# YzM1a0/MuDPT

Hardware: AMD Instinct MI355X
Metric: images/sec fwd+bwd ViT-B/16 MuDPT (higher is better)
Workload: dtype bf16; 1 GPU; MuDPT ViT-B/16 fwd+bwd+SGD, batch 256/GPU, 11 class prompts, n_ctx 4, depth 12, synthetic 224x224 N(0,1) images, random-init frozen CLIP (BASELINE configs[1]); global_batch=256, parallelism=dp1

## Files before the change

### include/mudpt.h

```cpp
#ifndef MUDPT_H
#define MUDPT_H

#include <stddef.h>
#include <stdint.h>

#ifdef __cplusplus
extern "C" {
#endif

#define MUDPT_ABI_VERSION 7

#define MUDPT_OK 0
#define MUDPT_ERR_ARG 1
#define MUDPT_ERR_HIP 2
#define MUDPT_ERR_STATE 3

#define MUDPT_BF16 0
#define MUDPT_F16 1
#define MUDPT_F32 2

#define MUDPT_VARIANT_MUDPT 0
#define MUDPT_VARIANT_COCOOP 1
#define MUDPT_VARIANT_COOP 2
#define MUDPT_VARIANT_COOP_CSC 3
// ... 141 lines not shown
int mudpt_cocoop_dbias(int32_t dtype, const float* dx_f32, const void* dx_lp, float* dbias, int32_t B, int32_t C, int32_t L, int32_t d,
                       int32_t n, float scale, void* stream);
int mudpt_coop_dctx(int32_t dtype, const float* dx_f32, const void* dx_lp, const int32_t* rows, float* dctx, int32_t C, int32_t n, int32_t d,
                    int32_t csc, float scale, void* stream);
int mudpt_sgemm(int32_t transA, int32_t transB, int32_t M, int32_t N, int32_t K, float alpha, const float* A, int32_t lda,
                const float* B, int32_t ldb, float beta, float* C, int32_t ldc, const float* bias, void* stream);

int mudpt_layernorm_bwd_ex(int32_t dtype, const void* dy, int32_t lddy, int32_t dy_f32, const float* x, int32_t ldx, const int32_t* row_index,
                           const float* mean, const float* rstd, const float* gamma, const float* dres, const void* dres_lp, int32_t lddres,
                           float* dx, int32_t lddx, void* dx_lp, int32_t lddx_lp, float* side, int32_t side_row0, int32_t side_n, int32_t side_L,
                           size_t side_ldb, int32_t index_mode, int32_t rows, int32_t d, void* stream);
int mudpt_layernorm_fwd_ex(int32_t dtype, const float* x, int32_t ldx, const int32_t* row_index, const float* add, const void* add_lp, int32_t ldadd,
                           const float* ov_rows, int32_t ov_row0, int32_t ov_n, int32_t ov_L, float* xout, int32_t ldxout, const float* gamma,
                           const float* beta, void* out, void* out_lo, int32_t lo_mode, int32_t ldo, int32_t out_f32, float* mean, float* rstd,
                           int32_t rows, int32_t d, void* stream);
int mudpt_attention_fwd_split(int32_t dtype, const void* qkv, void* out, void* out_lo, int32_t lo_mode, int32_t ld_out, float* lse, int32_t B, int32_t L,
                              int32_t H, int32_t causal, void* stream);
int mudpt_attention_fwd_single_split(int32_t dtype, const void* qkv, const void* q_sel, const int32_t* sel_rows, void* out_sel, void* out_lo,
                                     int32_t lo_mode, int32_t ld_out, float* lse_sel, int32_t B, int32_t L, int32_t H, int32_t causal, void* stream);
int mudpt_attention_bwd_sel(int32_t dtype, const void* qkv, const void* out, const void* dout, const float* lse, float* delta, void* dqkv,
                            const int32_t* sel_rows, int32_t B, int32_t L, int32_t H, int32_t causal, void* stream);
int mudpt_head_ex(const float* img, const float* txt, const int64_t* labels, float scale, float grad_scale, int32_t B, int32_t B_total, int32_t C,
                  int32_t e, float* txt_n, float* txt_inv, float* logits, float* loss, float* row_loss, float* dimg, float* dtxt, int32_t path,
                  int32_t* path_taken, void* stream);
int mudpt_pair_head(const float* img, const float* txt, const int64_t* labels, float scale, float grad_scale, int32_t B, int32_t B_total, int32_t C,
                    int32_t e, float* logits, float* loss, float* row_loss, float* dtxt, void* stream);
int mudpt_patchify(int32_t dtype, const float* images, void* patches, void* patches_lo, int32_t lo_mode, int32_t B, int32_t image_size, int32_t patch,
                   int32_t ldk, void* stream);
int mudpt_set_rows(float* x, int32_t B, int32_t L, int32_t d, int32_t row0, int32_t n, const float* rows, const float* add, void* stream);
int mudpt_gather_rows(const void* src, size_t src_stride, const int32_t* rows, void* dst, size_t dst_stride, int32_t nrows, int32_t row_bytes, void* stream);
// ... 31 lines not shown
```

### mudpt_amd/capi.py

```python
from __future__ import annotations

import ctypes as C
import os
import re

HERE = os.path.dirname(os.path.abspath(__file__))
LIB_PATH = os.environ.get("MUDPT_LIB") or os.path.join(HERE, "lib", "libmudpt_hip.so")
HEADER_PATH = os.path.join(os.path.dirname(HERE), "include", "mudpt.h")

BF16, F16, F32 = 0, 1, 2
VARIANT_MUDPT, VARIANT_COCOOP, VARIANT_COOP, VARIANT_COOP_CSC, VARIANT_VPT, VARIANT_MPT, VARIANT_UMUDPT, VARIANT_UUMUDPT = 0, 1, 2, 3, 4, 5, 6, 7
CLASS_TOKEN_END, CLASS_TOKEN_MIDDLE, CLASS_TOKEN_FRONT = 0, 1, 2
ABI_VERSION = 7
EPI_STORE, EPI_GELU, EPI_RESIDUAL, EPI_GELU_BWD, EPI_PATCH, EPI_STORE_F32 = range(6)
ATTN_FORMS = ("FWD_PAIR", "FWD_PERSISTENT", "FWD_RESIDENT", "FWD_STAGED", "BWD_TWO", "BWD_FUSED_W2", "BWD_FUSED_W1", "BWD_SWEEP", "BWD_RESIDENT",
              "BWD_STAGED")
GEMM_FORMS = ("PP", "T256x256", "T128x256", "T256x128", "T64x64_K128", "T64x64", "T128x64_RING4", "T128x128", "SPLITK_K128", "SPLITK_K64")


class MudptError(RuntimeError):
    pass


class Config(C.Structure):
# ... 55 lines not shown
    "mudpt_attention_fwd_exact": (_i32, [_vp, _vp, _vp, _vp, _i32, _i32, _vp, _i32, _i32, _i32, _i32, _vp]),
    "mudpt_attention_bwd": (_i32, [_i32, _vp, _vp, _vp, _vp, _vp, _vp, _i32, _i32, _i32, _i32, _vp]),
    "mudpt_attention_fwd_single": (_i32, [_i32, _vp, _vp, _vp, _vp, _vp, _i32, _i32, _i32, _i32, _vp]),
    "mudpt_attention_bwd_single": (_i32, [_i32, _vp, _vp, _vp, _vp, _vp, _vp, _vp, _vp, _i32, _i32, _i32, _i32, _vp]),
    "mudpt_layernorm_fwd_fused": (_i32, [_i32, _vp, _i32, _vp, _vp, _i32, _vp, _i32, _i32, _i32, _vp, _i32, _vp, _vp, _vp, _i32, _i32,
                                         _vp, _vp, _i32, _i32, _vp]),
    "mudpt_head": (_i32, [_vp, _vp, _vp, _f32, _f32, _i32, _i32, _i32, _vp, _vp, _vp, _vp, _vp]),
    "mudpt_reduce_rows": (_i32, [_i32, _vp, _vp, _i32, _i32, _i32, _i32, _i32, _vp, _i32, _i32, _f32, _vp]),
    "mudpt_cocoop_dbias": (_i32, [_i32, _vp, _vp, _vp, _i32, _i32, _i32, _i32, _i32, _f32, _vp]),
    "mudpt_coop_dctx": (_i32, [_i32, _vp, _vp, _vp, _vp, _i32, _i32, _i32, _i32, _f32, _vp]),
    "mudpt_sgemm": (_i32, [_i32, _i32, _i32, _i32, _i32, _f32, _vp, _i32, _vp, _i32, _f32, _vp, _i32, _vp, _vp]),
    "mudpt_layernorm_bwd_ex": (_i32, [_i32, _vp, _i32, _i32, _vp, _i32, _vp, _vp, _vp, _vp, _vp, _vp, _i32, _vp, _i32, _vp, _i32,
                                      _vp, _i32, _i32, _i32, _sz, _i32, _i32, _i32, _vp]),
    "mudpt_layernorm_fwd_ex": (_i32, [_i32, _vp, _i32, _vp, _vp, _vp, _i32, _vp, _i32, _i32, _i32, _vp, _i32, _vp, _vp, _vp, _vp, _i32, _i32, _i32,
                                      _vp, _vp, _i32, _i32, _vp]),
    "mudpt_attention_fwd_split": (_i32, [_i32, _vp, _vp, _vp, _i32, _i32, _vp, _i32, _i32, _i32, _i32, _vp]),
    "mudpt_attention_fwd_single_split": (_i32, [_i32, _vp, _vp, _vp, _vp, _vp, _i32, _i32, _vp, _i32, _i32, _i32, _i32, _vp]),
    "mudpt_attention_bwd_sel": (_i32, [_i32, _vp, _vp, _vp, _vp, _vp, _vp, _vp, _i32, _i32, _i32, _i32, _vp]),
    "mudpt_head_ex": (_i32, [_vp, _vp, _vp, _f32, _f32, _i32, _i32, _i32, _i32, _vp, _vp, _vp, _vp, _vp, _vp, _vp, _i32, C.POINTER(_i32), _vp]),
    "mudpt_pair_head": (_i32, [_vp, _vp, _vp, _f32, _f32, _i32, _i32, _i32, _i32, _vp, _vp, _vp, _vp, _vp]),
    "mudpt_patchify": (_i32, [_i32, _vp, _vp, _vp, _i32, _i32, _i32, _i32, _i32, _vp]),
    "mudpt_set_rows": (_i32, [_vp, _i32, _i32, _i32, _i32, _i32, _vp, _vp, _vp]),
    "mudpt_gather_rows": (_i32, [_vp, _sz, _vp, _vp, _sz, _i32, _i32, _vp]),
    "mudpt_scatter_rows": (_i32, [_vp, _sz, _vp, _vp, _sz, _i32, _i32, _vp]),
    "mudpt_add_rows": (_i32, [_i32, _vp, _vp, _vp, _i32, _i32, _vp]),
    "mudpt_linear_bwd": (_i32, [_i32, _i32, _i32, _vp, _vp, _vp, _vp, _vp, _vp, _vp]),
    "mudpt_colsum": (_i32, [_vp, _i32, _i32, _i32, _vp, _i32, _vp]),
    "mudpt_add": (_i32, [_vp, _vp, _vp, _sz, _vp]),
    "mudpt_cast": (_i32, [_i32, _vp, _vp, _sz, _vp]),
    "mudpt_relu": (_i32, [_vp, _sz, _vp]),
# ... 68 lines not shown
```

### mudpt_amd/csrc/common.h

```cpp
#pragma once
#include <hip/hip_runtime.h>
#include <hip/hip_ext.h>
#include <stdint.h>

#include "../../include/mudpt.h"

namespace mudpt {

typedef __attribute__((ext_vector_type(8))) __bf16 bf16x8;
typedef __attribute__((ext_vector_type(4))) __bf16 bf16x4;
typedef __attribute__((ext_vector_type(8))) _Float16 f16x8;
typedef __attribute__((ext_vector_type(4))) _Float16 f16x4;
typedef __attribute__((ext_vector_type(4))) float f32x4;
typedef __attribute__((ext_vector_type(16))) float f32x16;
typedef __attribute__((ext_vector_type(8))) int i32x8;

enum DType : int { DT_BF16 = 0, DT_F16 = 1 };

struct BF16 {
    using elem = __bf16;
    using vec8 = bf16x8;
    using vec4 = bf16x4;
    static constexpr int id = DT_BF16;
    __device__ static inline f32x4 mfma16(vec8 a, vec8 b, f32x4 c) {
// ... 71 lines not shown
}

template <int CTRL, int ROW_MASK = 0xf>
__device__ inline float dpp_mov(float v, float old) {
    return __builtin_bit_cast(float, __builtin_amdgcn_update_dpp(__builtin_bit_cast(int, old), __builtin_bit_cast(int, v), CTRL, ROW_MASK, 0xf, false));
}
__device__ inline float wave_sum(float v) {
    v += dpp_mov<0xb1>(v, 0.f);
    v += dpp_mov<0x4e>(v, 0.f);
    v += dpp_mov<0x141>(v, 0.f);
    v += dpp_mov<0x140>(v, 0.f);
    v += dpp_mov<0x142, 0xa>(v, 0.f);
    v += dpp_mov<0x143, 0xc>(v, 0.f);
    return __builtin_bit_cast(float, __builtin_amdgcn_readlane(__builtin_bit_cast(int, v), 63));
}
__device__ inline float wave_max(float v) {
    v = fmaxf(v, dpp_mov<0xb1>(v, v));
    v = fmaxf(v, dpp_mov<0x4e>(v, v));
    v = fmaxf(v, dpp_mov<0x141>(v, v));
    v = fmaxf(v, dpp_mov<0x140>(v, v));
    v = fmaxf(v, dpp_mov<0x142, 0xa>(v, v));
    v = fmaxf(v, dpp_mov<0x143, 0xc>(v, v));
    return __builtin_bit_cast(float, __builtin_amdgcn_readlane(__builtin_bit_cast(int, v), 63));
}

__device__ inline int xcd_remap(int bid, int nwg) {
    const int q = nwg >> 3, r = nwg & 7, x = bid & 7;
    return (x < r ? x * (q + 1) : r * (q + 1) + (x - r) * q) + (bid >> 3);
}

// ... 53 lines not shown
```

### mudpt_amd/csrc/kernels.h

```cpp
#pragma once
#include "common.h"

namespace mudpt {

enum Epilogue : int {
    EPI_STORE = 0,
    EPI_GELU = 1,
    EPI_RESIDUAL = 2,
    EPI_GELU_BWD = 3,
    EPI_PATCH = 4,
    EPI_STORE_F32 = 5
};

struct GemmArgs {
    const void* A = nullptr;
    const void* B = nullptr;
    int M = 0, N = 0, K = 0, lda = 0, ldb = 0;
    const float* bias = nullptr;
    void* out0 = nullptr; int ldo0 = 0;
    void* out1 = nullptr; int ldo1 = 0;
    void* out1_lo = nullptr;
    int out1_lo_mode = LO_F16;
    const void* A_lo = nullptr; int lo_mode = LO_NONE;
    const void* B8 = nullptr; int b8_scale = 127;
// ... 22 lines not shown
int launch_gemm_pp(int dtype, int epi, const GemmArgs& a, hipStream_t s, const GemmOpts& o);

struct LnFwdArgs {
    const float* x = nullptr; int ldx = 0;
    const int* row_index = nullptr;
    const float* gamma = nullptr; const float* beta = nullptr;
    void* out = nullptr; int ldo = 0;
    void* out_lo = nullptr;
    int lo_mode = LO_F16;
    float* mean = nullptr; float* rstd = nullptr;
    int rows = 0, d = 0; bool out_f32 = false;
    const float* add = nullptr; int ldadd = 0;
    const void* add_lp = nullptr;
    float* xout = nullptr; int ldxout = 0;
    const float* ov_rows = nullptr; int ov_row0 = 0, ov_n = 0, ov_L = 1;
};
int launch_ln_fwd(int dtype, const LnFwdArgs& a, hipStream_t s, const LaunchProf* prof = nullptr);

struct LnBwdArgs {
    const void* dy = nullptr; int lddy = 0; bool dy_f32 = false;
    const float* x = nullptr; int ldx = 0;
    const int* row_index = nullptr;
    const float* mean = nullptr; const float* rstd = nullptr; const float* gamma = nullptr;
    const float* dres = nullptr; int lddres = 0;
    const void* dres_lp = nullptr;
    float* dx = nullptr; int lddx = 0;
    void* dx_lp = nullptr; int lddx_lp = 0;
    int rows = 0, d = 0;
    bool by_token = false;
    bool stats_by_token = false;
// ... 130 lines not shown
```

### mudpt_amd/csrc/layernorm.hip

```cpp
#include "kernels.h"

namespace mudpt {

constexpr int LN_MAXV = 4;

template <typename T, bool OUT_F32>
__global__ __launch_bounds__(256) void ln_fwd_kernel(LnFwdArgs p) {
    using elem = typename T::elem;
    const int lane = threadIdx.x & 63;
    const int r = blockIdx.x * 4 + (threadIdx.x >> 6);
    if (r >= p.rows) return;
    const size_t xr = p.row_index ? (size_t)p.row_index[r] : (size_t)r;
    const f32x4* x = (const f32x4*)(p.x + xr * p.ldx);
    const int d4 = p.d >> 2;
    f32x4 v[LN_MAXV];
    float s = 0.f;
    const f32x4* ov = nullptr;
    if (p.ov_rows) {
        const int pos = r % p.ov_L - p.ov_row0;
        if (pos >= 0 && pos < p.ov_n) ov = (const f32x4*)(p.ov_rows + (size_t)pos * p.d);
    }
    const f32x4* add = (p.add && !ov) ? (const f32x4*)(p.add + xr * p.ldadd) : nullptr;
    const typename T::vec4* add_lp = (p.add_lp && !ov) ? (const typename T::vec4*)((const elem*)p.add_lp + xr * p.ldadd) : nullptr;
#pragma unroll
// ... 106 lines not shown
            for (int j = 0; j < 4; ++j) dx[j] = rstd * (g[k][j] - c1 - xh[k][j] * c2);
            if (p.dres) dx += ((const f32x4*)(p.dres + t * p.lddres))[i];
            if (p.dres_lp) {
                dx += f32x4{(float)rv[k][0], (float)rv[k][1], (float)rv[k][2], (float)rv[k][3]};
            }
            if (side_row) { side_row[i] = dx; dx = f32x4{0.f, 0.f, 0.f, 0.f}; }
            if (p.dx) ((f32x4*)(p.dx + t * p.lddx))[i] = dx;
            if (p.dx_lp) {
                typename T::vec4 o = {(elem)dx[0], (elem)dx[1], (elem)dx[2], (elem)dx[3]};
                ((typename T::vec4*)((elem*)p.dx_lp + t * p.lddx_lp))[i] = o;
            }
        }
    }
}

int launch_ln_fwd(int dtype, const LnFwdArgs& a, hipStream_t s, const LaunchProf* prof) {
    ARG_CHECK(a.x && a.gamma && a.beta && a.out, "ln_fwd: null operand");
    ARG_CHECK(a.rows > 0 && a.d > 0 && a.d % 4 == 0 && a.d <= 256 * LN_MAXV, "ln_fwd: bad shape rows=%d d=%d", a.rows, a.d);
    ARG_CHECK(a.ldx % 4 == 0 && a.ldo % 4 == 0 && a.ldx >= a.d && a.ldo >= a.d, "ln_fwd: bad strides %d/%d", a.ldx, a.ldo);
    ARG_CHECK(!(a.add || a.add_lp) || (a.ldadd % 4 == 0 && a.ldadd >= a.d), "ln_fwd: bad addend stride %d", a.ldadd);
    ARG_CHECK(!a.xout || (a.ldxout % 4 == 0 && a.ldxout >= a.d), "ln_fwd: bad xout stride %d", a.ldxout);
    ARG_CHECK(!a.ov_rows || (a.ov_L > 0 && a.ov_row0 >= 0 && a.ov_n >= 0 && a.ov_row0 + a.ov_n <= a.ov_L),
              "ln_fwd: bad splice rows %d..+%d of %d", a.ov_row0, a.ov_n, a.ov_L);
    ARG_CHECK(!a.row_index || !(a.add || a.add_lp || a.xout || a.ov_rows), "ln_fwd: the fused add / splice / xout need the identity row map");
    ARG_CHECK(!a.out_lo || (!a.out_f32 && (a.lo_mode == LO_F16 || a.lo_mode == LO_F8)), "ln_fwd: out_lo needs a T output and lo_mode 1 / 2");
    const dim3 grid((a.rows + 3) / 4), block(256);
    if (dtype == DT_BF16) {
        if (a.out_f32) MUDPT_LAUNCH((ln_fwd_kernel<BF16, true>), grid, block, 0, s, prof, a);
        else MUDPT_LAUNCH((ln_fwd_kernel<BF16, false>), grid, block, 0, s, prof, a);
    } else if (dtype == DT_F16) {
        if (a.out_f32) MUDPT_LAUNCH((ln_fwd_kernel<F16, true>), grid, block, 0, s, prof, a);
        else MUDPT_LAUNCH((ln_fwd_kernel<F16, false>), grid, block, 0, s, prof, a);
    } else {
        set_error("ln_fwd: unknown dtype %d", dtype);
        return MUDPT_ERR_ARG;
    }
    HIP_TRY(hipGetLastError());
    return MUDPT_OK;
}

int launch_ln_bwd(int dtype, const LnBwdArgs& a, hipStream_t s, const LaunchProf* prof) {
    ARG_CHECK(a.dy && a.x && a.mean && a.rstd && a.gamma && (a.dx || a.dx_lp), "ln_bwd: null operand");
    ARG_CHECK(!(a.dres && a.dres_lp), "ln_bwd: dres and dres_lp are exclusive");
    ARG_CHECK(!a.side || (!a.row_index && a.side_L > 0 && a.side_n > 0), "ln_bwd: the fused splice backward needs the identity row map");
    ARG_CHECK(a.rows > 0 && a.d > 0 && a.d % 4 == 0 && a.d <= 256 * LN_MAXV, "ln_bwd: bad shape rows=%d d=%d", a.rows, a.d);
    ARG_CHECK(a.ldx % 4 == 0 && a.lddy % 4 == 0 && a.lddx % 4 == 0, "ln_bwd: strides must be multiples of 4");
    ARG_CHECK(a.ldx >= a.d && a.lddy >= a.d && (!a.dx || a.lddx >= a.d), "ln_bwd: a row stride is shorter than d=%d (%d/%d/%d)", a.d, a.ldx, a.lddy, a.lddx);
    ARG_CHECK(!(a.dres || a.dres_lp) || (a.lddres % 4 == 0 && a.lddres >= a.d), "ln_bwd: bad dres stride %d", a.lddres);
    ARG_CHECK(!a.dx_lp || (a.lddx_lp % 4 == 0 && a.lddx_lp >= a.d), "ln_bwd: bad dx_lp stride %d", a.lddx_lp);
    ARG_CHECK(!a.side || (a.side_row0 >= 0 && a.side_row0 + a.side_n <= a.side_L && a.side_ldb % 4 == 0 && a.side_ldb >= (size_t)a.side_n * a.d),
              "ln_bwd: bad splice rows %d..+%d of %d / side stride %zu", a.side_row0, a.side_n, a.side_L, a.side_ldb);
    const dim3 grid((a.rows + 3) / 4), block(256);
    if (dtype == DT_BF16) {
        if (a.dy_f32) MUDPT_LAUNCH((ln_bwd_kernel<BF16, true>), grid, block, 0, s, prof, a);
        else MUDPT_LAUNCH((ln_bwd_kernel<BF16, false>), grid, block, 0, s, prof, a);
    } else if (dtype == DT_F16) {
        if (a.dy_f32) MUDPT_LAUNCH((ln_bwd_kernel<F16, true>), grid, block, 0, s, prof, a);
        else MUDPT_LAUNCH((ln_bwd_kernel<F16, false>), grid, block, 0, s, prof, a);
    } else {
        set_error("ln_bwd: unknown dtype %d", dtype);
        return MUDPT_ERR_ARG;
    }
    HIP_TRY(hipGetLastError());
    return MUDPT_OK;
}

}
```

### mudpt_amd/csrc/model.cpp

```cpp
#include <dlfcn.h>
#include <stdarg.h>
#include <stdio.h>
#include <string.h>

#include <algorithm>
#include <cmath>
#include <string>
#include <vector>

#include "../../include/mudpt.h"
#include "kernels.h"

namespace mudpt {

static thread_local char g_err[1024] = "";
void set_error(const char* fmt, ...) {
    va_list ap;
    va_start(ap, fmt);
    vsnprintf(g_err, sizeof(g_err), fmt, ap);
    va_end(ap);
}
const char* get_error() { return g_err; }

static inline uint16_t f32_to_bf16(float f) {
// ... 946 lines not shown
    if (m_fc != LO_NONE) { l2.out_lo = t.h_sel_lo; l2.lo_mode = m_fc; }
    TRY(launch_ln_fwd(dt, l2, s));
    GemmArgs f; f.A = t.h_sel; f.lda = d; f.B = w.w_fc; f.ldb = d; f.M = S; f.N = 4 * d; f.K = d; f.bias = w.b_fc;
    split_operand(f, m_fc, t.h_sel_lo, w.w_fc8, w.s_fc8);
    f.out0 = t.u_sel; f.ldo0 = 4 * d; f.out1 = t.g_sel; f.ldo1 = 4 * d;
    f.gelu_q8 = m->gelu_q8 && t.split == LO_NONE;
    if (m_proj != LO_NONE) { f.out1_lo = t.g_sel_lo; f.out1_lo_mode = m_proj; }
    TRY(gemm_call(m, EPI_GELU, f, s));
    GemmArgs p; p.A = t.g_sel; p.lda = 4 * d; p.B = w.w_proj; p.ldb = 4 * d; p.M = S; p.N = d; p.K = 4 * d; p.bias = w.b_proj;
    split_operand(p, m_proj, t.g_sel_lo, w.w_proj8, w.s_proj8);
    p.out0 = t.xout_sel; p.ldo0 = d; p.aux = t.xmid_sel; p.ldaux = d;
    TRY(gemm_call(m, EPI_RESIDUAL, p, s));
    return MUDPT_OK;
}

static int block_fwd(mudpt_model* m, Tower& t, int i, int nseq, const float* splice, hipStream_t s) {
    const int M = tower_rows(t, nseq), d = t.d, dt = m->dtype, n = t.n;
    const std::vector<Tower::Seg> segs = tower_segs(t, nseq);
    const bool lp = m->lp_upd;
    BlockW& w = t.w[i];
    BlockAct& a = t.a[i];
    const size_t esz = 2;
    const int m_qkv = site_mode(t, SITE_QKV, d), m_out = site_mode(t, SITE_OUT, d), m_fc = site_mode(t, SITE_FC, d), m_proj = site_mode(t, SITE_PROJ, 4 * d);
    LnFwdArgs l1; l1.x = a.x_in; l1.ldx = d; l1.gamma = w.ln1_g; l1.beta = w.ln1_b; l1.out = t.h; l1.ldo = d; l1.mean = a.mean1; l1.rstd = a.rstd1; l1.rows = M; l1.d = d;
    if (m_qkv != LO_NONE) { l1.out_lo = t.h_lo; l1.lo_mode = m_qkv; }
    if (i > 0) {
        l1.x = t.a[i - 1].x_mid; l1.ldadd = d; l1.xout = a.x_in; l1.ldxout = d;
        if (lp) l1.add_lp = t.upd; else l1.add = t.upd;
        if (splice) { l1.ov_rows = splice; l1.ov_row0 = t.prompt_row0; l1.ov_n = n; l1.ov_L = t.L; }
    }
    if (splice && i > 0 && segs.size() > 1) {
        for (const Tower::Seg& g : segs) {
            LnFwdArgs b = l1;
            const size_t r0 = (size_t)g.row0;
            b.x = l1.x + r0 * l1.ldx; b.xout = l1.xout + r0 * l1.ldxout;
            if (l1.add) b.add = l1.add + r0 * l1.ldadd;
            if (l1.add_lp) b.add_lp = (const char*)l1.add_lp + r0 * l1.ldadd * esz;
            b.out = (char*)l1.out + r0 * l1.ldo * esz;
            if (l1.out_lo) b.out_lo = (char*)l1.out_lo + r0 * l1.ldo * esz;
            b.mean = l1.mean + r0; b.rstd = l1.rstd + r0; b.rows = g.nseq * g.L; b.ov_L = g.L;
            TRY(ln_fwd_call(m, t, b, s));
        }
    } else {
        TRY(ln_fwd_call(m, t, l1, s));
    }
    if (i + 1 == t.layers && m->last_single && !t.exact_attn && t.tail_rows) {
// ... 190 lines not shown
    const mudpt_config& c = m->cfg;
    const int dv = c.v_width, e = c.embed_dim, n = m->vis.n, D1 = m->vis.D1;
    const int P = (c.image_size / c.patch) * (c.image_size / c.patch), Lv = m->vis.L, K0 = (3 * c.patch * c.patch + 63) / 64 * 64;
    const PromptRoute pr = prompt_route(m, m->vis);
    const int m_patch = site_mode(m->vis, SITE_PATCH, K0);
    if (m_patch != LO_NONE) TRY(launch_patchify_split(m->dtype, images, m->patches, m->patches_lo, m_patch, B, c.image_size, c.patch, K0, s));
    else TRY(launch_patchify(m->dtype, images, m->patches, B, c.image_size, c.patch, K0, s));
    GemmArgs pe; pe.A = m->patches; pe.lda = K0; pe.B = m->conv_w; pe.ldb = K0; pe.M = B * P; pe.N = dv; pe.K = K0; pe.out0 = m->xpre; pe.ldo0 = dv;
    split_operand(pe, m_patch, m->patches_lo, m->conv_w8, m->conv_s8);
    pe.patches = P; pe.seq_len = Lv; pe.pos = m->vpos;
    TRY(gemm_call(m, EPI_PATCH, pe, s));
    TRY(launch_set_rows(m->xpre, B, Lv, dv, 0, 1, m->cls, m->vpos, s));
    if (n > 0) TRY(launch_set_rows(m->xpre, B, Lv, dv, Lv - n, n, pr.in0, pr.in0_add, s));
    LnFwdArgs lp; lp.x = m->xpre; lp.ldx = dv; lp.gamma = m->ln_pre_g; lp.beta = m->ln_pre_b; lp.out = m->vis.a[0].x_in; lp.ldo = dv; lp.out_f32 = true;
    lp.mean = m->pre_mean; lp.rstd = m->pre_rstd; lp.rows = B * Lv; lp.d = dv;
    TRY(launch_ln_fwd(m->dtype, lp, s));
    for (int i = 0; i < m->vis.layers; ++i) {
        TRY(block_fwd(m, m->vis, i, B, (i >= 1 && i - 1 < D1) ? pr.deep + (size_t)(i - 1) * n * dv : nullptr, s));
    }
    LnFwdArgs lq; lq.x = m->vis.xout_sel; lq.ldx = dv; lq.gamma = m->ln_post_g; lq.beta = m->ln_post_b; lq.out = m->f_ln; lq.ldo = dv;
    lq.out_f32 = true; lq.mean = m->post_mean; lq.rstd = m->post_rstd; lq.rows = B; lq.d = dv;
    TRY(launch_ln_fwd(m->dtype, lq, s));
    TRY(launch_sgemm(false, false, B, e, dv, 1.f, m->f_ln, dv, m->vproj, e, 0.f, m->img_f, e, nullptr, s));
    return MUDPT_OK;
}

static int cocoop_text_chunk(mudpt_model* m, int i0, int nb, hipStream_t s) {
    const mudpt_config& c = m->cfg;
    const int dt = c.t_width, e = c.embed_dim, n = c.n_ctx, C = c.n_cls, Lt = m->txt.L, TS = nb * C;
    const size_t r0 = (size_t)i0 * C;
    TRY(launch_cocoop_prompts(m->txt.a[0].x_in, m->emb_pos, m->params + m->off(Q_CTX), m->mn_bias + (size_t)i0 * dt, m->tpos, nb, C, Lt, dt, n, s));
    for (int i = 0; i < m->txt.layers; ++i) TRY(block_fwd(m, m->txt, i, TS, nullptr, s));
    LnFwdArgs lf; lf.x = m->txt.xout_sel; lf.ldx = dt; lf.gamma = m->ln_fin_g; lf.beta = m->ln_fin_b; lf.out = m->t_ln + r0 * dt; lf.ldo = dt;
// ... 783 lines not shown
    a.dres = dres; a.dres_lp = dres_lp; a.lddres = lddres; a.dx = dx; a.lddx = lddx; a.dx_lp = dx_lp; a.lddx_lp = lddx_lp; a.rows = rows; a.d = d;
    a.by_token = index_mode == 1; a.stats_by_token = index_mode == 2;
    if (side) { a.side = side; a.side_row0 = side_row0; a.side_n = side_n; a.side_L = side_L; a.side_ldb = side_ldb; }
    return launch_ln_bwd(dtype, a, (hipStream_t)stream);
}
extern "C" int mudpt_layernorm_fwd_ex(int32_t dtype, const float* x, int32_t ldx, const int32_t* row_index, const float* add, const void* add_lp, int32_t ldadd,
                                      const float* ov_rows, int32_t ov_row0, int32_t ov_n, int32_t ov_L, float* xout, int32_t ldxout, const float* gamma,
                                      const float* beta, void* out, void* out_lo, int32_t lo_mode, int32_t ldo, int32_t out_f32, float* mean, float* rstd,
                                      int32_t rows, int32_t d, void* stream) {
    LnFwdArgs a; a.x = x; a.ldx = ldx; a.row_index = row_index; a.add = add; a.add_lp = add_lp; a.ldadd = ldadd; a.xout = xout; a.ldxout = ldxout;
    a.gamma = gamma; a.beta = beta; a.out = out; a.out_lo = out_lo; a.lo_mode = lo_mode; a.ldo = ldo; a.out_f32 = out_f32 != 0; a.mean = mean; a.rstd = rstd;
    a.rows = rows; a.d = d;
    if (ov_rows) { a.ov_rows = ov_rows; a.ov_row0 = ov_row0; a.ov_n = ov_n; a.ov_L = ov_L; }
    return launch_ln_fwd(dtype, a, (hipStream_t)stream);
}
extern "C" int mudpt_attention_fwd_split(int32_t dtype, const void* qkv, void* out, void* out_lo, int32_t lo_mode, int32_t ld_out, float* lse, int32_t B, int32_t L,
                                         int32_t H, int32_t causal, void* stream) {
    AttnArgs a; a.qkv = qkv; a.out = out; a.out_lo = out_lo; a.lo_mode = lo_mode; a.ld_out = ld_out; a.lse = lse; a.B = B; a.L = L; a.H = H;
    const AttnOpts o = attn_flags(causal, false, a);
    return launch_attn_fwd(dtype, a, (hipStream_t)stream, o);
}
extern "C" int mudpt_attention_fwd_single_split(int32_t dtype, const void* qkv, const void* q_sel, const int32_t* sel_rows, void* out_sel, void* out_lo,
                                                int32_t lo_mode, int32_t ld_out, float* lse_sel, int32_t B, int32_t L, int32_t H, int32_t causal, void* stream) {
    AttnArgs a; a.qkv = qkv; a.sel_rows = sel_rows; a.lo_mode = lo_mode; a.B = B; a.L = L; a.H = H; a.causal = causal != 0;
    return launch_attn_fwd_single(dtype, a, q_sel, out_sel, out_lo, ld_out, lse_sel, (hipStream_t)stream);
}
extern "C" int mudpt_attention_bwd_sel(int32_t dtype, const void* qkv, const void* out, const void* dout, const float* lse, float* delta, void* dqkv,
                                       const int32_t* sel_rows, int32_t B, int32_t L, int32_t H, int32_t causal, void* stream) {
    ARG_CHECK(sel_rows, "attention_bwd_sel: null sel_rows");
    AttnArgs a; a.qkv = qkv; a.out = (void*)out; a.dout = dout; a.lse = (float*)lse; a.delta = delta; a.dqkv = dqkv; a.sel_rows = sel_rows; a.B = B; a.L = L; a.H = H;
// ... 122 lines not shown
```

Before: 10720 images/s.

## Add register-resident wide LayerNorm kernels and fuse ln_pre with first block ln1

Adds wide LayerNorm forward and backward kernels that keep a whole row in registers across a half-wave. Each lane handles 8 contiguous elements per 256-wide chunk and reduces with DPP half-wave sums. These kernels are used whenever d is a multiple of 256 and the low-precision rows are aligned. Adds a two-norm kernel that applies ln_pre and the first block's ln1 in one pass, writing the f32 residual plus the low-precision (and optional lo-split) QKV input, so block 0 skips its own LN launch. This removes one kernel launch and one full read/write of the activation, at the cost of more template variants and more register pressure.

```diff
diff --git a/include/mudpt.h b/include/mudpt.h
--- a/include/mudpt.h
+++ b/include/mudpt.h
@@ -179,6 +179,9 @@
                            const float* ov_rows, int32_t ov_row0, int32_t ov_n, int32_t ov_L, float* xout, int32_t ldxout, const float* gamma,
                            const float* beta, void* out, void* out_lo, int32_t lo_mode, int32_t ldo, int32_t out_f32, float* mean, float* rstd,
                            int32_t rows, int32_t d, void* stream);
+int mudpt_layernorm_fwd_pair(int32_t dtype, const float* x, int32_t ldx, const float* gamma, const float* beta, float* xout, int32_t ldxout, float* mean,
+                             float* rstd, const float* gamma2, const float* beta2, void* out, void* out_lo, int32_t lo_mode, int32_t ldo, float* mean2,
+                             float* rstd2, int32_t rows, int32_t d, void* stream);
 int mudpt_attention_fwd_split(int32_t dtype, const void* qkv, void* out, void* out_lo, int32_t lo_mode, int32_t ld_out, float* lse, int32_t B, int32_t L,
                               int32_t H, int32_t causal, void* stream);
 int mudpt_attention_fwd_single_split(int32_t dtype, const void* qkv, const void* q_sel, const int32_t* sel_rows, void* out_sel, void* out_lo,
diff --git a/mudpt_amd/capi.py b/mudpt_amd/capi.py
--- a/mudpt_amd/capi.py
+++ b/mudpt_amd/capi.py
@@ -93,6 +93,7 @@
                                       _vp, _i32, _i32, _i32, _sz, _i32, _i32, _i32, _vp]),
     "mudpt_layernorm_fwd_ex": (_i32, [_i32, _vp, _i32, _vp, _vp, _vp, _i32, _vp, _i32, _i32, _i32, _vp, _i32, _vp, _vp, _vp, _vp, _i32, _i32, _i32,
                                       _vp, _vp, _i32, _i32, _vp]),
+    "mudpt_layernorm_fwd_pair": (_i32, [_i32, _vp, _i32, _vp, _vp, _vp, _i32, _vp, _vp, _vp, _vp, _vp, _vp, _i32, _i32, _vp, _vp, _i32, _i32, _vp]),
     "mudpt_attention_fwd_split": (_i32, [_i32, _vp, _vp, _vp, _i32, _i32, _vp, _i32, _i32, _i32, _i32, _vp]),
     "mudpt_attention_fwd_single_split": (_i32, [_i32, _vp, _vp, _vp, _vp, _vp, _i32, _i32, _vp, _i32, _i32, _i32, _i32, _vp]),
     "mudpt_attention_bwd_sel": (_i32, [_i32, _vp, _vp, _vp, _vp, _vp, _vp, _vp, _i32, _i32, _i32, _i32, _vp]),
diff --git a/mudpt_amd/csrc/common.h b/mudpt_amd/csrc/common.h
--- a/mudpt_amd/csrc/common.h
+++ b/mudpt_amd/csrc/common.h
@@ -109,6 +109,16 @@
     v += dpp_mov<0x143, 0xc>(v, 0.f);
     return __builtin_bit_cast(float, __builtin_amdgcn_readlane(__builtin_bit_cast(int, v), 63));
 }
+__device__ inline float halfwave_sum(float v) {
+    v += dpp_mov<0xb1>(v, 0.f);
+    v += dpp_mov<0x4e>(v, 0.f);
+    v += dpp_mov<0x141>(v, 0.f);
+    v += dpp_mov<0x140>(v, 0.f);
+    v += dpp_mov<0x142, 0xa>(v, 0.f);
+    const float lo = __builtin_bit_cast(float, __builtin_amdgcn_readlane(__builtin_bit_cast(int, v), 31));
+    const float hi = __builtin_bit_cast(float, __builtin_amdgcn_readlane(__builtin_bit_cast(int, v), 63));
+    return (threadIdx.x & 32) ? hi : lo;
+}
 __device__ inline float wave_max(float v) {
     v = fmaxf(v, dpp_mov<0xb1>(v, v));
     v = fmaxf(v, dpp_mov<0x4e>(v, v));
diff --git a/mudpt_amd/csrc/kernels.h b/mudpt_amd/csrc/kernels.h
--- a/mudpt_amd/csrc/kernels.h
+++ b/mudpt_amd/csrc/kernels.h
@@ -60,6 +60,8 @@
     const void* add_lp = nullptr;
     float* xout = nullptr; int ldxout = 0;
     const float* ov_rows = nullptr; int ov_row0 = 0, ov_n = 0, ov_L = 1;
+    const float* gamma2 = nullptr; const float* beta2 = nullptr;
+    float* mean2 = nullptr; float* rstd2 = nullptr;
 };
 int launch_ln_fwd(int dtype, const LnFwdArgs& a, hipStream_t s, const LaunchProf* prof = nullptr);
 
diff --git a/mudpt_amd/csrc/layernorm.hip b/mudpt_amd/csrc/layernorm.hip
--- a/mudpt_amd/csrc/layernorm.hip
+++ b/mudpt_amd/csrc/layernorm.hip
@@ -1,3 +1,7 @@
+#include <initializer_list>
+#include <type_traits>
+#include <utility>
+
 #include "kernels.h"
 
 namespace mudpt {
@@ -144,6 +148,286 @@
     }
 }
 
+#pragma clang fp contract(off)
+
+constexpr int LN_W = 8;
+
+__device__ inline void ld_f32(float (&v)[LN_W], const float* p) {
+#pragma unroll
+    for (int q = 0; q < LN_W / 4; ++q) {
+        const f32x4 t = ((const f32x4*)p)[q];
+#pragma unroll
+        for (int j = 0; j < 4; ++j) v[4 * q + j] = t[j];
+    }
+}
+__device__ inline void st_f32(float* p, const float (&v)[LN_W]) {
+#pragma unroll
+    for (int q = 0; q < LN_W / 4; ++q) ((f32x4*)p)[q] = f32x4{v[4 * q], v[4 * q + 1], v[4 * q + 2], v[4 * q + 3]};
+}
+template <typename E>
+using lpvec = __attribute__((ext_vector_type(LN_W))) E;
+template <typename E>
+__device__ inline void st_lp(E* p, const E (&v)[LN_W]) {
+    lpvec<E> o;
+#pragma unroll
+    for (int j = 0; j < LN_W; ++j) o[j] = v[j];
+    *(lpvec<E>*)p = o;
+}
+
+template <int NCH>
+__device__ inline void ln_stats(const float (&v)[NCH][LN_W], int d, float& mean, float& rstd) {
+    float sa = 0.f, sb = 0.f;
+#pragma unroll
+    for (int k = 0; k < NCH; ++k) {
+        sa += v[k][0] + v[k][1] + v[k][2] + v[k][3];
+        sb += v[k][4] + v[k][5] + v[k][6] + v[k][7];
+    }
+    mean = halfwave_sum(sa + sb) / d;
+    float qa = 0.f, qb = 0.f;
+#pragma unroll
+    for (int k = 0; k < NCH; ++k) {
+#pragma unroll
+        for (int j = 0; j < 4; ++j) {
+            const float ca = v[k][j] - mean, cb = v[k][4 + j] - mean;
+            qa += ca * ca;
+            qb += cb * cb;
+        }
+    }
+    rstd = rsqrtf(halfwave_sum(qa + qb) / d + 1e-5f);
+}
+template <typename T, bool OUT_F32>
+__device__ inline void ln_emit(const LnFwdArgs& p, int r, int e, const float (&y)[LN_W]) {
+    using elem = typename T::elem;
+    if constexpr (OUT_F32) {
+        st_f32((float*)p.out + (size_t)r * p.ldo + e, y);
+    } else {
+        elem o[LN_W];
+        if (p.out_lo) {
+            elem lo[LN_W];
+            float rem[LN_W];
+#pragma unroll
+            for (int j = 0; j < LN_W; ++j) { rem[j] = split_rem(y[j], o[j]); lo[j] = (elem)rem[j]; }
+            if (p.lo_mode == LO_F8) *(uint2*)((char*)p.out_lo + (size_t)r * p.ldo * 2 + e) = uint2{pack_lo8(rem[0], rem[1], rem[2], rem[3]), pack_lo8(rem[4], rem[5], rem[6], rem[7])};
+            else st_lp((elem*)p.out_lo + (size_t)r * p.ldo + e, lo);
+        } else {
+#pragma unroll
+            for (int j = 0; j < LN_W; ++j) o[j] = (elem)y[j];
+        }
+        st_lp((elem*)p.out + (size_t)r * p.ldo + e, o);
+    }
+}
+
+template <typename T, bool OUT_F32, int NCH>
+__global__ __launch_bounds__(256) void ln_fwd_wide_kernel(LnFwdArgs p) {
+    using elem = typename T::elem;
+    const int e0 = LN_W * (threadIdx.x & 31);
+    const int r = (blockIdx.x * 256 + threadIdx.x) >> 5;
+    if (r >= p.rows) return;
+    const size_t xr = p.row_index ? (size_t)p.row_index[r] : (size_t)r;
+    const float* src = p.x + xr * p.ldx;
+    const float* add = p.add ? p.add + xr * p.ldadd : nullptr;
+    const elem* add_lp = p.add_lp ? (const elem*)p.add_lp + xr * p.ldadd : nullptr;
+    bool ov = false;
+    if (p.ov_rows) {
+        const int pos = r % p.ov_L - p.ov_row0;
+        if (pos >= 0 && pos < p.ov_n) {
+            ov = true;
+            src = p.ov_rows + (size_t)pos * p.d;
+            add = src;
+            add_lp = (const elem*)src;
+        }
+    }
+    float v[NCH][LN_W];
+#pragma unroll
+    for (int k = 0; k < NCH; ++k) ld_f32(v[k], src + 256 * k + e0);
+    if (p.add) {
+        float a[NCH][LN_W];
+#pragma unroll
+        for (int k = 0; k < NCH; ++k) ld_f32(a[k], add + 256 * k + e0);
+#pragma unroll
+        for (int k = 0; k < NCH; ++k) {
+#pragma unroll
+            for (int j = 0; j < LN_W; ++j) v[k][j] = ov ? v[k][j] : v[k][j] + a[k][j];
+        }
+    }
+    if (p.add_lp) {
+        lpvec<elem> a[NCH];
+#pragma unroll
+        for (int k = 0; k < NCH; ++k) a[k] = *(const lpvec<elem>*)(add_lp + 256 * k + e0);
+#pragma unroll
+        for (int k = 0; k < NCH; ++k) {
+#pragma unroll
+            for (int j = 0; j < LN_W; ++j) v[k][j] = ov ? v[k][j] : v[k][j] + (float)a[k][j];
+        }
+    }
+    float g[NCH][LN_W], b[NCH][LN_W];
+#pragma unroll
+    for (int k = 0; k < NCH; ++k) {
+        ld_f32(g[k], p.gamma + 256 * k + e0);
+        ld_f32(b[k], p.beta + 256 * k + e0);
+    }
+    if (p.xout) {
+#pragma unroll
+        for (int k = 0; k < NCH; ++k) st_f32(p.xout + xr * p.ldxout + 256 * k + e0, v[k]);
+    }
+    float mean, rstd;
+    ln_stats(v, p.d, mean, rstd);
+    if (e0 == 0) {
+        if (p.mean) p.mean[r] = mean;
+        if (p.rstd) p.rstd[r] = rstd;
+    }
+#pragma unroll
+    for (int k = 0; k < NCH; ++k) {
+        float y[LN_W];
+#pragma unroll
+        for (int j = 0; j < LN_W; ++j) y[j] = __builtin_fmaf((v[k][j] - mean) * rstd, g[k][j], b[k][j]);
+        ln_emit<T, OUT_F32>(p, r, 256 * k + e0, y);
+    }
+}
+
+template <typename T, int NCH>
+__global__ __launch_bounds__(256) void ln_fwd_pair_kernel(LnFwdArgs p) {
+    const int e0 = LN_W * (threadIdx.x & 31);
+    const int r = (blockIdx.x * 256 + threadIdx.x) >> 5;
+    if (r >= p.rows) return;
+    float v[NCH][LN_W], g[NCH][LN_W], b[NCH][LN_W];
+#pragma unroll
+    for (int k = 0; k < NCH; ++k) {
+        ld_f32(v[k], p.x + (size_t)r * p.ldx + 256 * k + e0);
+        ld_f32(g[k], p.gamma + 256 * k + e0);
+        ld_f32(b[k], p.beta + 256 * k + e0);
+    }
+    float mean, rstd;
+    ln_stats(v, p.d, mean, rstd);
+#pragma unroll
+    for (int k = 0; k < NCH; ++k) {
+#pragma unroll
+        for (int j = 0; j < LN_W; ++j) v[k][j] = __builtin_fmaf((v[k][j] - mean) * rstd, g[k][j], b[k][j]);
+        ld_f32(g[k], p.gamma2 + 256 * k + e0);
+        ld_f32(b[k], p.beta2 + 256 * k + e0);
+    }
+#pragma unroll
+    for (int k = 0; k < NCH; ++k) st_f32(p.xout + (size_t)r * p.ldxout + 256 * k + e0, v[k]);
+    float mean2, rstd2;
+    ln_stats(v, p.d, mean2, rstd2);
+    if (e0 == 0) {
+        if (p.mean) p.mean[r] = mean;
+        if (p.rstd) p.rstd[r] = rstd;
+        if (p.mean2) p.mean2[r] = mean2;
+        if (p.rstd2) p.rstd2[r] = rstd2;
+    }
+#pragma unroll
+    for (int k = 0; k < NCH; ++k) {
+        float y[LN_W];
+#pragma unroll
+        for (int j = 0; j < LN_W; ++j) y[j] = __builtin_fmaf((v[k][j] - mean2) * rstd2, g[k][j], b[k][j]);
+        ln_emit<T, false>(p, r, 256 * k + e0, y);
+    }
+}
+
+template <typename T, bool DY_F32, int NCH>
+__global__ __launch_bounds__(256) void ln_bwd_wide_kernel(LnBwdArgs p) {
+    using elem = typename T::elem;
+    const int e0 = LN_W * (threadIdx.x & 31);
+    const int r = (blockIdx.x * 256 + threadIdx.x) >> 5;
+    if (r >= p.rows) return;
+    const size_t t = p.row_index ? (size_t)p.row_index[r] : (size_t)r;
+    const size_t sr = p.by_token ? t : (size_t)r;
+    const size_t st = (p.by_token || p.stats_by_token) ? t : (size_t)r;
+    const float mean = p.mean[st], rstd = p.rstd[st];
+    float* side_row = nullptr;
+    if (p.side) {
+        const int pos = (int)(t % (size_t)p.side_L) - p.side_row0;
+        if (pos >= 0 && pos < p.side_n) side_row = p.side + (t / (size_t)p.side_L) * p.side_ldb + (size_t)pos * p.d;
+    }
+    float xh[NCH][LN_W], g[NCH][LN_W];
+    lpvec<elem> rv[NCH];
+#pragma unroll
+    for (int k = 0; k < NCH; ++k) {
+        ld_f32(g[k], p.gamma + 256 * k + e0);
+        ld_f32(xh[k], p.x + t * p.ldx + 256 * k + e0);
+    }
+    if (p.dres_lp) {
+#pragma unroll
+        for (int k = 0; k < NCH; ++k) rv[k] = *(const lpvec<elem>*)((const elem*)p.dres_lp + t * p.lddres + 256 * k + e0);
+    }
+    float s1[2] = {0.f, 0.f}, s2[2] = {0.f, 0.f};
+    {
+        std::conditional_t<DY_F32, float, lpvec<elem>> dy[NCH][DY_F32 ? LN_W : 1];
+#pragma unroll
+        for (int k = 0; k < NCH; ++k) {
+            if constexpr (DY_F32) ld_f32(dy[k], (const float*)p.dy + sr * p.lddy + 256 * k + e0);
+            else dy[k][0] = *(const lpvec<elem>*)((const elem*)p.dy + sr * p.lddy + 256 * k + e0);
+        }
+#pragma unroll
+        for (int k = 0; k < NCH; ++k) {
+#pragma unroll
+            for (int j = 0; j < LN_W; ++j) {
+                float dv;
+                if constexpr (DY_F32) dv = dy[k][j];
+                else dv = (float)dy[k][0][j];
+                xh[k][j] = (xh[k][j] - mean) * rstd;
+                g[k][j] = dv * g[k][j];
+                s1[j >> 2] += g[k][j];
+                s2[j >> 2] += g[k][j] * xh[k][j];
+            }
+        }
+    }
+    const float c1 = halfwave_sum(s1[0] + s1[1]) / p.d, c2 = halfwave_sum(s2[0] + s2[1]) / p.d;
+#pragma unroll
+    for (int k = 0; k < NCH; ++k) {
+        const int e = 256 * k + e0;
+        float dx[LN_W];
+#pragma unroll
+        for (int j = 0; j < LN_W; ++j) dx[j] = rstd * __builtin_fmaf(-xh[k][j], c2, g[k][j] - c1);
+        if (p.dres) {
+            float a[LN_W];
+            ld_f32(a, p.dres + t * p.lddres + e);
+#pragma unroll
+            for (int j = 0; j < LN_W; ++j) dx[j] += a[j];
+        }
+        if (p.dres_lp) {
+#pragma unroll
+            for (int j = 0; j < LN_W; ++j) dx[j] += (float)rv[k][j];
+        }
+        if (side_row) {
+            st_f32(side_row + e, dx);
+#pragma unroll
+            for (int j = 0; j < LN_W; ++j) dx[j] = 0.f;
+        }
+        if (p.dx) st_f32(p.dx + t * p.lddx + e, dx);
+        if (p.dx_lp) {
+            elem o[LN_W];
+#pragma unroll
+            for (int j = 0; j < LN_W; ++j) o[j] = (elem)dx[j];
+            st_lp((elem*)p.dx_lp + t * p.lddx_lp + e, o);
+        }
+    }
+}
+
+static bool ln_wide(int d, std::initializer_list<std::pair<const void*, int>> lp_rows) {
+    if (d % 256) return false;
+    for (const auto& o : lp_rows)
+        if (o.first && (((uintptr_t)o.first & 15) || o.second % 8)) return false;
+    return true;
+}
+
+#define LN_LAUNCH_WIDE(d, KERN, ...)                                                                                             \
+    do {                                                                                                                         \
+        const dim3 grid((a.rows + 7) / 8), block(256);                                                                           \
+        if (dtype == DT_BF16) {                                                                                                  \
+            if ((d) == 256) MUDPT_LAUNCH((KERN<BF16, ##__VA_ARGS__, 1>), grid, block, 0, s, prof, a);                            \
+            else if ((d) == 512) MUDPT_LAUNCH((KERN<BF16, ##__VA_ARGS__, 2>), grid, block, 0, s, prof, a);                       \
+            else if ((d) == 768) MUDPT_LAUNCH((KERN<BF16, ##__VA_ARGS__, 3>), grid, block, 0, s, prof, a);                       \
+            else MUDPT_LAUNCH((KERN<BF16, ##__VA_ARGS__, 4>), grid, block, 0, s, prof, a);                                       \
+        } else {                                                                                                                 \
+            if ((d) == 256) MUDPT_LAUNCH((KERN<F16, ##__VA_ARGS__, 1>), grid, block, 0, s, prof, a);                             \
+            else if ((d) == 512) MUDPT_LAUNCH((KERN<F16, ##__VA_ARGS__, 2>), grid, block, 0, s, prof, a);                        \
+            else if ((d) == 768) MUDPT_LAUNCH((KERN<F16, ##__VA_ARGS__, 3>), grid, block, 0, s, prof, a);                        \
+            else MUDPT_LAUNCH((KERN<F16, ##__VA_ARGS__, 4>), grid, block, 0, s, prof, a);                                        \
+        }                                                                                                                        \
+    } while (0)
+
 int launch_ln_fwd(int dtype, const LnFwdArgs& a, hipStream_t s, const LaunchProf* prof) {
     ARG_CHECK(a.x && a.gamma && a.beta && a.out, "ln_fwd: null operand");
     ARG_CHECK(a.rows > 0 && a.d > 0 && a.d % 4 == 0 && a.d <= 256 * LN_MAXV, "ln_fwd: bad shape rows=%d d=%d", a.rows, a.d);
@@ -154,16 +438,25 @@
               "ln_fwd: bad splice rows %d..+%d of %d", a.ov_row0, a.ov_n, a.ov_L);
     ARG_CHECK(!a.row_index || !(a.add || a.add_lp || a.xout || a.ov_rows), "ln_fwd: the fused add / splice / xout need the identity row map");
     ARG_CHECK(!a.out_lo || (!a.out_f32 && (a.lo_mode == LO_F16 || a.lo_mode == LO_F8)), "ln_fwd: out_lo needs a T output and lo_mode 1 / 2");
-    const dim3 grid((a.rows + 3) / 4), block(256);
-    if (dtype == DT_BF16) {
-        if (a.out_f32) MUDPT_LAUNCH((ln_fwd_kernel<BF16, true>), grid, block, 0, s, prof, a);
-        else MUDPT_LAUNCH((ln_fwd_kernel<BF16, false>), grid, block, 0, s, prof, a);
-    } else if (dtype == DT_F16) {
-        if (a.out_f32) MUDPT_LAUNCH((ln_fwd_kernel<F16, true>), grid, block, 0, s, prof, a);
-        else MUDPT_LAUNCH((ln_fwd_kernel<F16, false>), grid, block, 0, s, prof, a);
+    ARG_CHECK(dtype == DT_BF16 || dtype == DT_F16, "ln_fwd: unknown dtype %d", dtype);
+    const bool wide = ln_wide(a.d, {{a.add_lp, a.ldadd}, {a.out_f32 ? nullptr : a.out, a.ldo}, {a.lo_mode == LO_F8 ? nullptr : a.out_lo, a.ldo}});
+    if (a.gamma2) {
+        ARG_CHECK(a.beta2 && a.xout && !a.out_f32 && !(a.add || a.add_lp || a.ov_rows || a.row_index),
+                  "ln_fwd: the two-norm form takes beta2 and xout, a T output and no add / splice / row map");
+        ARG_CHECK(wide, "ln_fwd: the two-norm form needs d %% 256 == 0 and 16-byte aligned T rows (d=%d ldo=%d)", a.d, a.ldo);
+        LN_LAUNCH_WIDE(a.d, ln_fwd_pair_kernel);
+    } else if (wide) {
+        if (a.out_f32) LN_LAUNCH_WIDE(a.d, ln_fwd_wide_kernel, true);
+        else LN_LAUNCH_WIDE(a.d, ln_fwd_wide_kernel, false);
     } else {
-        set_error("ln_fwd: unknown dtype %d", dtype);
-        return MUDPT_ERR_ARG;
+        const dim3 grid((a.rows + 3) / 4), block(256);
+        if (dtype == DT_BF16) {
+            if (a.out_f32) MUDPT_LAUNCH((ln_fwd_kernel<BF16, true>), grid, block, 0, s, prof, a);
+            else MUDPT_LAUNCH((ln_fwd_kernel<BF16, false>), grid, block, 0, s, prof, a);
+        } else {
+            if (a.out_f32) MUDPT_LAUNCH((ln_fwd_kernel<F16, true>), grid, block, 0, s, prof, a);
+            else MUDPT_LAUNCH((ln_fwd_kernel<F16, false>), grid, block, 0, s, prof, a);
+        }
     }
     HIP_TRY(hipGetLastError());
     return MUDPT_OK;
@@ -180,19 +473,23 @@
     ARG_CHECK(!a.dx_lp || (a.lddx_lp % 4 == 0 && a.lddx_lp >= a.d), "ln_bwd: bad dx_lp stride %d", a.lddx_lp);
     ARG_CHECK(!a.side || (a.side_row0 >= 0 && a.side_row0 + a.side_n <= a.side_L && a.side_ldb % 4 == 0 && a.side_ldb >= (size_t)a.side_n * a.d),
               "ln_bwd: bad splice rows %d..+%d of %d / side stride %zu", a.side_row0, a.side_n, a.side_L, a.side_ldb);
-    const dim3 grid((a.rows + 3) / 4), block(256);
-    if (dtype == DT_BF16) {
-        if (a.dy_f32) MUDPT_LAUNCH((ln_bwd_kernel<BF16, true>), grid, block, 0, s, prof, a);
-        else MUDPT_LAUNCH((ln_bwd_kernel<BF16, false>), grid, block, 0, s, prof, a);
-    } else if (dtype == DT_F16) {
-        if (a.dy_f32) MUDPT_LAUNCH((ln_bwd_kernel<F16, true>), grid, block, 0, s, prof, a);
-        else MUDPT_LAUNCH((ln_bwd_kernel<F16, false>), grid, block, 0, s, prof, a);
+    ARG_CHECK(dtype == DT_BF16 || dtype == DT_F16, "ln_bwd: unknown dtype %d", dtype);
+    if (ln_wide(a.d, {{a.dy_f32 ? nullptr : a.dy, a.lddy}, {a.dres_lp, a.lddres}, {a.dx_lp, a.lddx_lp}})) {
+        if (a.dy_f32) LN_LAUNCH_WIDE(a.d, ln_bwd_wide_kernel, true);
+        else LN_LAUNCH_WIDE(a.d, ln_bwd_wide_kernel, false);
     } else {
-        set_error("ln_bwd: unknown dtype %d", dtype);
-        return MUDPT_ERR_ARG;
+        const dim3 grid((a.rows + 3) / 4), block(256);
+        if (dtype == DT_BF16) {
+            if (a.dy_f32) MUDPT_LAUNCH((ln_bwd_kernel<BF16, true>), grid, block, 0, s, prof, a);
+            else MUDPT_LAUNCH((ln_bwd_kernel<BF16, false>), grid, block, 0, s, prof, a);
+        } else {
+            if (a.dy_f32) MUDPT_LAUNCH((ln_bwd_kernel<F16, true>), grid, block, 0, s, prof, a);
+            else MUDPT_LAUNCH((ln_bwd_kernel<F16, false>), grid, block, 0, s, prof, a);
+        }
     }
     HIP_TRY(hipGetLastError());
     return MUDPT_OK;
 }
-
-}
+#undef LN_LAUNCH_WIDE
+
+}
diff --git a/mudpt_amd/csrc/model.cpp b/mudpt_amd/csrc/model.cpp
--- a/mudpt_amd/csrc/model.cpp
+++ b/mudpt_amd/csrc/model.cpp
@@ -984,7 +984,7 @@
     return MUDPT_OK;
 }
 
-static int block_fwd(mudpt_model* m, Tower& t, int i, int nseq, const float* splice, hipStream_t s) {
+static int block_fwd(mudpt_model* m, Tower& t, int i, int nseq, const float* splice, hipStream_t s, bool h_ready = false) {
     const int M = tower_rows(t, nseq), d = t.d, dt = m->dtype, n = t.n;
     const std::vector<Tower::Seg> segs = tower_segs(t, nseq);
     const bool lp = m->lp_upd;
@@ -999,7 +999,8 @@
         if (lp) l1.add_lp = t.upd; else l1.add = t.upd;
         if (splice) { l1.ov_rows = splice; l1.ov_row0 = t.prompt_row0; l1.ov_n = n; l1.ov_L = t.L; }
     }
-    if (splice && i > 0 && segs.size() > 1) {
+    if (h_ready) {
+    } else if (splice && i > 0 && segs.size() > 1) {
         for (const Tower::Seg& g : segs) {
             LnFwdArgs b = l1;
             const size_t r0 = (size_t)g.row0;
@@ -1220,9 +1221,18 @@
     if (n > 0) TRY(launch_set_rows(m->xpre, B, Lv, dv, Lv - n, n, pr.in0, pr.in0_add, s));
     LnFwdArgs lp; lp.x = m->xpre; lp.ldx = dv; lp.gamma = m->ln_pre_g; lp.beta = m->ln_pre_b; lp.out = m->vis.a[0].x_in; lp.ldo = dv; lp.out_f32 = true;
     lp.mean = m->pre_mean; lp.rstd = m->pre_rstd; lp.rows = B * Lv; lp.d = dv;
-    TRY(launch_ln_fwd(m->dtype, lp, s));
+    const bool pair = !m->cocoop && m->vis.layers > 1 && dv % 256 == 0;
+    if (pair) {
+        const int m_qkv = site_mode(m->vis, SITE_QKV, dv);
+        lp.out_f32 = false; lp.xout = m->vis.a[0].x_in; lp.ldxout = dv; lp.out = m->vis.h;
+        lp.gamma2 = m->vis.w[0].ln1_g; lp.beta2 = m->vis.w[0].ln1_b; lp.mean2 = m->vis.a[0].mean1; lp.rstd2 = m->vis.a[0].rstd1;
+        if (m_qkv != LO_NONE) { lp.out_lo = m->vis.h_lo; lp.lo_mode = m_qkv; }
+        TRY(ln_fwd_call(m, m->vis, lp, s));
+    } else {
+        TRY(launch_ln_fwd(m->dtype, lp, s));
+    }
     for (int i = 0; i < m->vis.layers; ++i) {
-        TRY(block_fwd(m, m->vis, i, B, (i >= 1 && i - 1 < D1) ? pr.deep + (size_t)(i - 1) * n * dv : nullptr, s));
+        TRY(block_fwd(m, m->vis, i, B, (i >= 1 && i - 1 < D1) ? pr.deep + (size_t)(i - 1) * n * dv : nullptr, s, pair && i == 0));
     }
     LnFwdArgs lq; lq.x = m->vis.xout_sel; lq.ldx = dv; lq.gamma = m->ln_post_g; lq.beta = m->ln_post_b; lq.out = m->f_ln; lq.ldo = dv;
     lq.out_f32 = true; lq.mean = m->post_mean; lq.rstd = m->post_rstd; lq.rows = B; lq.d = dv;
@@ -2036,6 +2046,15 @@
     if (ov_rows) { a.ov_rows = ov_rows; a.ov_row0 = ov_row0; a.ov_n = ov_n; a.ov_L = ov_L; }
     return launch_ln_fwd(dtype, a, (hipStream_t)stream);
 }
+extern "C" int mudpt_layernorm_fwd_pair(int32_t dtype, const float* x, int32_t ldx, const float* gamma, const float* beta, float* xout, int32_t ldxout,
+                                        float* mean, float* rstd, const float* gamma2, const float* beta2, void* out, void* out_lo, int32_t lo_mode,
+                                        int32_t ldo, float* mean2, float* rstd2, int32_t rows, int32_t d, void* stream) {
+    ARG_CHECK(gamma2 && beta2, "layernorm_fwd_pair: needs gamma2 and beta2");
+    LnFwdArgs a; a.x = x; a.ldx = ldx; a.gamma = gamma; a.beta = beta; a.xout = xout; a.ldxout = ldxout; a.mean = mean; a.rstd = rstd;
+    a.gamma2 = gamma2; a.beta2 = beta2; a.out = out; a.out_lo = out_lo; if (out_lo) a.lo_mode = lo_mode; a.ldo = ldo; a.mean2 = mean2; a.rstd2 = rstd2;
+    a.rows = rows; a.d = d;
+    return launch_ln_fwd(dtype, a, (hipStream_t)stream);
+}
 extern "C" int mudpt_attention_fwd_split(int32_t dtype, const void* qkv, void* out, void* out_lo, int32_t lo_mode, int32_t ld_out, float* lse, int32_t B, int32_t L,
                                          int32_t H, int32_t causal, void* stream) {
     AttnArgs a; a.qkv = qkv; a.out = out; a.out_lo = out_lo; a.lo_mode = lo_mode; a.ld_out = ld_out; a.lse = lse; a.B = B; a.L = L; a.H = H;
```

Result: no change. 10790 images/s, median of 6 (+0.6%).
